# csyxwei/FFWM

Hardware: AMD Instinct MI355X
Metric: train img/s (128x128, full FFWM GAN step) (higher is better)
Workload: dtype f32; 1 GPU; BASELINE configs[2]: full FFWM train step (netG+netD+flowNetF+flowNetB, all losses, 3x Adam), synthetic MultiPIE-shaped 128x128; batch_per_gpu=8, global_batch=8, parallelism=dp1, grad_buckets=10, bucket_MiB=64

## Files before the change

### ffwm_amd/_lib.py

```python
import ctypes
import os

_HERE = os.path.dirname(os.path.abspath(__file__))
LIB_PATH = os.path.join(_HERE, "lib", "libffwm_hip.so")

F32, F64 = 0, 1
ABI_VERSION = 5

_lib = None

_p = ctypes.c_void_p
_i64 = ctypes.c_int64
_i = ctypes.c_int

_SIGNATURES = {
    "ffwm_block_extractor_forward": [_p, _p, _p] + [_i64] * 6 + [_i, _i, _p],
    "ffwm_block_extractor_backward": [_p, _p, _p, _p, _p] + [_i64] * 6 + [_i, _i, _p],
    "ffwm_block_extractor_backward_strided": [_p, _p, _p, ctypes.POINTER(_i64), _p, _p] + [_i64] * 6 + [_i, _i, _p],
    "ffwm_local_attn_reshape_backward_strided": [_p, ctypes.POINTER(_i64), _p] + [_i64] * 3 + [_i, _i, _i, _p],
    "ffwm_resample2d_backward_strided": [_p, _p, _p, ctypes.POINTER(_i64), _p, _p] + [_i64] * 6 + [_i, _i, _i, _i, _p],
    "ffwm_bn_lrelu_forward": [_p] * 9 + [_i64] * 3 + [ctypes.c_double] * 3 + [_i, _p],
    "ffwm_bn_lrelu_backward": [_p] * 10 + [_i64] * 3 + [ctypes.c_double] + [_i, _p],
    "ffwm_bn_res_act_forward": [_p] * 11 + [_i64] * 3 + [ctypes.c_double] * 3 + [_i, _i, _p],
    "ffwm_bn_res_act_backward": [_p] * 11 + [_i64] * 3 + [ctypes.c_double] + [_i, _i, _p],
    "ffwm_mfm_forward": [_p, _p, _p] + [_i64] * 3 + [_i, _p],
    "ffwm_mfm_backward": [_p, _p, _p, _p] + [_i64] * 3 + [_i, _p],
    "ffwm_add_act_forward": [_p, _p, _p, _i64, _i, ctypes.c_double, _i, _p],
    "ffwm_add_act_backward": [_p, _p, _p, _i64, _i, ctypes.c_double, _i, _p],
    "ffwm_sigmoid_gate_forward": [_p, _p, _p, _p, _p, _i64, _i, _p],
    "ffwm_sigmoid_gate_backward": [_p, _p, _p, _p, _p, _i64, _i, _p],
    "ffwm_bias_relu_forward": [_p, _p, _p] + [_i64] * 3 + [_i, _p],
    "ffwm_bias_act_forward": [_p, _p, _p, _p] + [_i64] * 5 + [_i, ctypes.c_double, _i, _p],
    "ffwm_flow_head_forward": [_p, _p, _p, _p] + [_i64] * 4 + [_i, _p],
    "ffwm_conv_thin_forward": [_p, _p, _p, _p] + [_i64] * 5 + [_i, ctypes.c_double, _i, _p],
    "ffwm_flow_up_forward": [_p, _p, _p, _p] + [_i64] * 4 + [_i, _p],
    "ffwm_flow_head_backward": [_p, _p, _p, _p, _p] + [_i64] * 4 + [_i, _p],
    "ffwm_flow_up_backward": [_p, _p, _p] + [_i64] * 4 + [_i, _p],
    "ffwm_conv2d_forward": [_p, _p, _p, _p, _p] + [_i64] * 5 + [_i, _i, _i, _i, _i64, _i64, _i, ctypes.c_double, _p, _i64, _i, _p],
    "ffwm_conv2d_wgrad": [_p, _p, _p] + [_i64] * 7 + [_i, _i, _i, _i, _p],
    "ffwm_conv2d_wgrad_tiled": [_p, _p, _p, _p] + [_i64] * 7 + [_i, _i, _i, _i, _i, _p],
    "ffwm_conv3x3_winograd_forward": [_p, _p, _p, _p, _p] + [_i64] * 5 + [_i, _i, ctypes.c_double, _i, _p],
    "ffwm_adam_step": [_p, _p, _p, _p, _i64] + [ctypes.c_double] * 4 + [_i64, _i, _p],
    "ffwm_adam_step_device": [_p, _p, _p, _p, _i64] + [ctypes.c_double] * 4 + [_p, _i, _p],
    "ffwm_conv3x3_wgrad": [_p, _p, _p, _p] + [_i64] * 5 + [_i, _p],
    "ffwm_conv3x3_wgrad_block": [_p, _p, _p, _p] + [_i64] * 9 + [_i, _p],
    "ffwm_block_attention_forward": [_p, _p, _p, _p] + [_i64] * 6 + [_i, _i, _p],
    "ffwm_block_attention_backward": [_p, _p, _p, _p, _p, _p, _p] + [_i64] * 6 + [_i, _i, _p],
    "ffwm_local_attn_reshape_forward": [_p, _p] + [_i64] * 3 + [_i, _i, _p],
    "ffwm_local_attn_reshape_backward": [_p, _p] + [_i64] * 3 + [_i, _i, _i, _p],
    "ffwm_resample2d_forward": [_p, _p, _p] + [_i64] * 6 + [_i, _i, _i, _p],
    "ffwm_resample2d_backward": [_p, _p, _p, _p, _p] + [_i64] * 6 + [_i, _i, _i, _i, _p],
    "ffwm_warp_forward": [_p, _p, _p] + [_i64] * 6 + [_i, _i, _p],
    "ffwm_warp_backward": [_p, _p, _p, _p, _p] + [_i64] * 6 + [_i, _i, _p],
    "ffwm_warp_multi_forward": [_p, _i, _i, _i, _p],
    "ffwm_warp_multi_backward": [_p, _i, _i, _i, _p],
    "ffwm_spectral_norm_forward": [_p, _i, _i, ctypes.c_double, _i, _p],
    "ffwm_spectral_norm_backward": [_p, _i, _i, _p],
    "ffwm_guided_filter_forward": [_p, _p, _p, _p, _i64, _i64, _i64, _i, ctypes.c_double, _i, _p],
    "ffwm_affine_regularization": [_p, _p, _p, _p, _i64, _i64, _i64, _i, ctypes.c_double, _i, _p],
    "ffwm_correlation_colmax": [_p, _p, _p, _i64, _i64, _i64, _i, _p],
    "ffwm_guided_filter_backward": [_p, _p, _p, _p, _p, _p, _i64, _i64, _i64, _i, _i, _p],
    "ffwm_l1_multi": [_p, _i, _p, _p, _i, _i, _p],
    "ffwm_conv3x3_winograd_weights_multi": [_p, _i, _i, _p],
    "ffwm_prof_enable": [_i],
    "ffwm_prof_collect": [],
    "ffwm_prof_get": [_i, ctypes.c_char_p, _i, ctypes.POINTER(_i64), ctypes.POINTER(ctypes.c_double),
                      ctypes.POINTER(ctypes.c_double)],
    "ffwm_prof_get_flops": [_i, ctypes.POINTER(ctypes.c_double)],
    "ffwm_prof_get_bound": [_i, ctypes.POINTER(ctypes.c_double)],
    "ffwm_prof_reset": [],
    "ffwm_set_option": [ctypes.c_char_p, _i],
    "ffwm_zero_fill": [_p, _i64, _p],
    "ffwm_abi_version": [],
}

EXPORTS = sorted(list(_SIGNATURES) + ["ffwm_last_error", "ffwm_conv3x3_winograd_workspace_bytes", "ffwm_conv3x3_winograd_splits",
                                      "ffwm_conv2d_forward_workspace"])


class FFWMError(RuntimeError):
    pass


def load():
    global _lib
    if _lib is not None:
        return _lib
    if not os.path.exists(LIB_PATH):
        raise FFWMError(
            "libffwm_hip.so is missing (%s). The HIP extension is the only implementation of the "
            "ffwm_amd ops -- build it with `python -m ffwm_amd.build`." % LIB_PATH)
    lib = ctypes.CDLL(LIB_PATH)
    for name, argtypes in _SIGNATURES.items():
        fn = getattr(lib, name)
        fn.argtypes = argtypes
        fn.restype = _i
    lib.ffwm_conv3x3_winograd_workspace_bytes.argtypes = [_i64, _i64]
    lib.ffwm_conv3x3_winograd_workspace_bytes.restype = _i64
    lib.ffwm_conv3x3_winograd_splits.argtypes = [_i64, _i64, _i64, _i64, _i64, _i]
    lib.ffwm_conv3x3_winograd_splits.restype = _i
    lib.ffwm_conv2d_forward_workspace.argtypes = [_i64] * 5 + [_i] * 4
    lib.ffwm_conv2d_forward_workspace.restype = _i64
    lib.ffwm_last_error.argtypes = []
    lib.ffwm_last_error.restype = ctypes.c_char_p
    got = lib.ffwm_abi_version()
    if got != ABI_VERSION:
        raise FFWMError("libffwm_hip.so ABI version %d, expected %d: rebuild it" % (got, ABI_VERSION))
    _lib = lib
    for kv in filter(None, os.environ.get("FFWM_OPTS", "").split(",")):
        k, _, v = kv.partition("=")
        if lib.ffwm_set_option(k.strip().encode(), int(v)) < 0:
            raise FFWMError("FFWM_OPTS: unknown option %r (or a negative value)" % k)
    return lib


def check(rc, what):
    if rc != 0:
        msg = load().ffwm_last_error()
        raise FFWMError("%s failed (status %d): %s" % (what, rc, msg.decode() if msg else "?"))


def prof_enable(on=True):
    return load().ffwm_prof_enable(1 if on else 0)


def prof_reset():
    load().ffwm_prof_reset()


def prof_collect():
    lib = load()
    n = lib.ffwm_prof_collect()
    rows = {}
    for i in range(n):
        name = ctypes.create_string_buffer(128)
        launches = _i64()
        ms = ctypes.c_double()
        nbytes = ctypes.c_double()
        check(lib.ffwm_prof_get(i, name, 128, ctypes.byref(launches), ctypes.byref(ms),
                                ctypes.byref(nbytes)), "ffwm_prof_get")
        flops = ctypes.c_double()
        check(lib.ffwm_prof_get_flops(i, ctypes.byref(flops)), "ffwm_prof_get_flops")
        bound = ctypes.c_double()
        check(lib.ffwm_prof_get_bound(i, ctypes.byref(bound)), "ffwm_prof_get_bound")
        k = max(launches.value, 1)
        rows[name.value.decode()] = {"launches": launches.value, "total_ms": ms.value,
                                     "avg_ms": ms.value / k, "bytes_per_launch": nbytes.value / k,
                                     "flops_per_launch": flops.value / k, "roofline_ms": bound.value}
    return rows


def set_option(key, value):
    rc = load().ffwm_set_option(key.encode(), int(value))
    if rc < 0:
        check(rc, "ffwm_set_option")
    return rc
```

### ffwm_amd/nets.py

```python
import math
import os

import torch
import torch.nn as nn
import torch.nn.functional as F
from torch.nn.utils import spectral_norm

from . import _ext
from . import conv as _conv
from .external_function import WarpFlipCat, WarpNet, warp_many

LRELU = 0.2


def _msra(mods):
    for m in mods:
        if isinstance(m, (nn.Conv2d, nn.ConvTranspose2d)):
            nn.init.kaiming_normal_(m.weight)
            if m.bias is not None:
                nn.init.constant_(m.bias, 0)


def _cbl(cin, cout, stride=1):
    return nn.Sequential(nn.Conv2d(cin, cout, 3, stride, 1, bias=True), nn.BatchNorm2d(cout),
                         nn.LeakyReLU(LRELU, inplace=True))


def _dbl(cin, cout):
    return nn.Sequential(nn.ConvTranspose2d(cin, cout, 4, 2, 1, bias=True), nn.BatchNorm2d(cout),
                         nn.LeakyReLU(LRELU, inplace=True))


def _flow_head(cin):
    return nn.Sequential(nn.Conv2d(cin, 2, 3, 1, 1, bias=True), nn.Tanh())


class FlowNet(nn.Module):

    def __init__(self, ngf=64, in_ch=3, keep_unused=True):
        super().__init__()
        g = ngf
        enc = [("conv0", in_ch, g, 1), ("conv1", g, g, 2), ("conv1_1", g, 2 * g, 1),
               ("conv2", 2 * g, 2 * g, 2), ("conv2_1", 2 * g, 2 * g, 1), ("conv3", 2 * g, 4 * g, 2),
               ("conv3_1", 4 * g, 4 * g, 1), ("conv4", 4 * g, 8 * g, 2), ("conv4_1", 8 * g, 8 * g, 1),
               ("conv5", 8 * g, 8 * g, 2), ("conv5_1", 8 * g, 8 * g, 1), ("conv6", 8 * g, 16 * g, 2),
               ("conv6_1", 16 * g, 16 * g, 1)]
        for name, cin, cout, s in enc:
            setattr(self, name, _cbl(cin, cout, s))
        cat = {5: 16 * g + 2, 4: 12 * g + 2, 3: 6 * g + 2, 2: g + 2, 1: g // 2 + 2, 0: g // 4 + 2}
        dec_out = {5: 8 * g, 4: 4 * g, 3: 2 * g, 2: g, 1: g // 2, 0: g // 4}
        dec_in = {5: 16 * g, 4: cat[5], 3: cat[4], 2: cat[3], 1: cat[2], 0: cat[1]}
        for L in range(5, -1, -1):
            setattr(self, "deconv%d" % L, _dbl(dec_in[L], dec_out[L]))
        for L in range(5, -1, -1):
            setattr(self, "inter_conv%d" % L, _cbl(cat[L], dec_out[L]))
        if keep_unused:
            for L in range(5, -1, -1):
                setattr(self, "inter_conv_occ%d" % L, _cbl(cat[L] - 1, dec_out[L]))
        heads = {6: 16 * g, 5: 8 * g, 4: 4 * g, 3: 2 * g, 2: g, 1: g // 2, 0: g // 4}
        for L in range(6, -1, -1):
            setattr(self, "predict_flow%d" % L, _flow_head(heads[L]))
        for L in range(6, 0, -1):
            setattr(self, "upsampled_flow%d_to_%d" % (L, L - 1), nn.ConvTranspose2d(2, 2, 4, 2, 1))
        _msra(self.modules())

    def unused_parameters(self):
        return [p for n, p in self.named_parameters() if n.startswith("inter_conv_occ")]

    def forward(self, x):
        f = self.conv0(x)
        skips = {}
        for L in range(1, 7):
            f = getattr(self, "conv%d_1" % L)(getattr(self, "conv%d" % L)(f))
            skips[L] = f
        flow = self.predict_flow6(f)
        flows = {}
        cat = None
        for L in range(5, -1, -1):
            up = getattr(self, "upsampled_flow%d_to_%d" % (L + 1, L))(flow)
            d = getattr(self, "deconv%d" % L)(f if L == 5 else cat)
            cat = torch.cat((skips[L], d, up) if L >= 3 else (d, up), 1)
            flow = getattr(self, "predict_flow%d" % L)(getattr(self, "inter_conv%d" % L)(cat))
            flows[L] = flow
        return flows[0], flows[1], flows[2]


class Tanh2(nn.Module):
    def forward(self, x):
        return (torch.tanh(x) + 1) / 2


def _activ(name):
    table = {"relu": nn.ReLU, "lrelu": lambda: nn.LeakyReLU(LRELU), "sigmoid": nn.Sigmoid, "tanh": nn.Tanh,
             "tanh2": Tanh2}
    if name not in table:
        raise NotImplementedError("Activation %s not implemented" % name)
    return table[name]()


def _sn(m, on):
    return spectral_norm(m) if on else m


class ResidualBlock(nn.Module):

    def __init__(self, inc, outc=None, kernel=3, activ="lrelu", sn=True):
        super().__init__()
        outc = inc if outc is None else outc
        pad = kernel // 2 if sn else kernel
        self.activ = _activ(activ)
        self.input = _sn(nn.Conv2d(inc, outc, 1, 1, 0), sn)
        self.blocks = nn.Sequential(_sn(nn.Conv2d(inc, outc, kernel, 1, pad), sn), nn.BatchNorm2d(outc),
                                    nn.LeakyReLU(LRELU), _sn(nn.Conv2d(outc, outc, kernel, 1, pad), sn),
                                    nn.BatchNorm2d(outc))

    def forward(self, x):
        return self.activ(self.blocks(x) + self.input(x))


class FusedResidualBlock(ResidualBlock):

    def forward(self, x):
        from .norm import RES_ACTS, bn_res_act, bn_res_act_ok
        from .residual import _act_of, add_act
        blocks, inp = self.blocks, self.input
        bn = blocks[-1] if isinstance(blocks, nn.Sequential) and len(blocks) >= 2 else None
        act, slope = _act_of(self.activ)
        if (bn is not None and isinstance(inp, nn.Conv2d) and not inp._forward_pre_hooks and not inp._forward_hooks
                and bn_res_act_ok(bn, x, RES_ACTS.get(act)) and torch.is_grad_enabled()):
            h = x
            for m in list(blocks)[:-1]:
                h = m(h)
            s = inp._conv_forward(x, inp.weight, None)
            if h.shape == s.shape and h.shape[1] == bn.num_features:
                return bn_res_act(h, bn, s, inp.bias, RES_ACTS[act], slope)
            return add_act(bn(h), s if inp.bias is None else s + inp.bias.view(1, -1, 1, 1), self.activ)
        return add_act(blocks(x), inp(x), self.activ)


def _conv_block(inc, outc, ks, s, p, activ="lrelu", res=0, bn=True, sn=True):
    layers = [_sn(nn.Conv2d(inc, outc, ks, s, p), sn)]
    if bn:
        layers.append(nn.BatchNorm2d(outc))
    if activ is not None:
        layers.append(_activ(activ))
    layers += [ResidualBlock(outc, activ=activ, sn=sn) for _ in range(res)]
    return nn.Sequential(*layers)


def _shuffle_block(inc, outc, sn=True):
    return nn.Sequential(_sn(nn.Conv2d(inc, outc * 4, 3, 1, 1), sn), nn.PixelShuffle(2), nn.BatchNorm2d(outc),
                         _activ("lrelu"))


class FFWM(nn.Module):

    def __init__(self, num_layers=3, isflip=True, sn=True, warp_flipcat=None):
        super().__init__()
        ch = [64, 64, 128, 256]
        dch = [256, 128, 64, 64]
        self.isflip = isflip
        dm = 3 if isflip else 2
        am = dm - 1
        self.layers = num_layers
        self.e0 = _conv_block(3, ch[0], 7, 1, 3, res=1, bn=False, sn=sn)
        for i in (1, 2, 3):
            setattr(self, "e%d" % i, _conv_block(ch[i - 1], ch[i], 4, 2, 1, res=1, sn=sn))
        d_in = [dch[0], dch[1] * dm, dch[2] * dm + 3]
        r_ch = [dch[1] * dm, dch[2] * dm + 3, dch[3] * dm + 3]
        for i in range(3):
            setattr(self, "d%d" % i, _shuffle_block(d_in[i], dch[i + 1], sn=sn))
        for i in range(3):
            setattr(self, "dres%d" % i, nn.Sequential(*[ResidualBlock(r_ch[i], activ="lrelu", sn=sn) for _ in range(2)]))
        for i in range(3):
            setattr(self, "rec%d" % i, _conv_block(r_ch[i], 3, 3, 1, 1, bn=False, activ="sigmoid", sn=sn))
        for i, c in enumerate((ch[2] * am, ch[1] * am, ch[0] * am)):
            setattr(self, "att%d" % i, nn.Sequential(_conv_block(c, c, 3, 1, 1, sn=sn),
                                                     ResidualBlock(c, c, activ="sigmoid", sn=sn)))
        self.warpNet = WarpNet()
        self._fused = warp_flipcat if warp_flipcat is not None else WarpFlipCat()
        self._multi = warp_flipcat is None and os.environ.get("FFWM_WARP_MULTI", "1") != "0"
        self.fuse_gate = False

    def _skip(self, feat, flow):
        if self.isflip:
            return self._fused(feat, flow)
        return self.warpNet(feat, flow)

    def _skips(self, enc, flow):
        feats = [enc[self.layers - 1 - i] for i in range(self.layers)]
        if self._multi and feats[0].is_cuda:
            return warp_many(feats, [flow[i] for i in range(self.layers)], self.isflip)
        return [self._skip(f, flow[i]) for i, f in enumerate(feats)]

    def forward(self, x, flow=None, return_att=False):
        enc = [self.e0(x)]
        for i in range(1, self.layers + 1):
            enc.append(getattr(self, "e%d" % i)(enc[-1]))
        fdec = enc[-1]
        recons, att = [], None
        if callable(flow):
            flow = flow()
        skips = self._skips(enc, flow) if self._multi else None
        for i in range(self.layers):
            dec = getattr(self, "d%d" % i)(fdec)
            skip = skips[i] if skips is not None else self._skip(enc[self.layers - 1 - i], flow[i])
            if self.fuse_gate:
                from .residual import gated
                skip, att = gated(getattr(self, "att%d" % i), skip)
            else:
                att = getattr(self, "att%d" % i)(skip)
                skip = skip * att
            parts = [skip, dec]
            if recons:
                parts.append(F.interpolate(recons[-1], scale_factor=2, mode="bilinear"))
            fdec = getattr(self, "dres%d" % i)(torch.cat(parts, 1))
            recons.append(getattr(self, "rec%d" % i)(fdec))
        out = (recons[-3], recons[-2], recons[-1])
        return out + (att,) if return_att else out


class WarpAttention(nn.Module):

    LEVELS = ((128, 32), (64, 64), (64, 128))

    def __init__(self, sn=True, warp_flipcat=None):
        super().__init__()
        for i, (c, _) in enumerate(self.LEVELS):
            setattr(self, "att%d" % i, nn.Sequential(_conv_block(2 * c, 2 * c, 3, 1, 1, sn=sn),
                                                     ResidualBlock(2 * c, 2 * c, activ="sigmoid", sn=sn)))
        self._fused = warp_flipcat if warp_flipcat is not None else WarpFlipCat()
        self._multi = warp_flipcat is None
        self.fuse_gate = False

    def forward(self, feats, flows):
        if self._multi and feats[0].is_cuda:
            skips = warp_many(list(feats), list(flows), True)
        else:
            skips = [self._fused(feat, flow) for feat, flow in zip(feats, flows)]
        if self.fuse_gate:
            from .residual import gated
            return [gated(getattr(self, "att%d" % i), skip)[0] for i, skip in enumerate(skips)]
        return [skip * getattr(self, "att%d" % i)(skip) for i, skip in enumerate(skips)]


class MSDiscriminator(nn.Module):

    def __init__(self, real_crop_size=128, inc=3, max_n_scales=9, scale_factor=2, base_channels=64, sigmoid=False):
        super().__init__()
        self.scale_factor = scale_factor
        n = int(math.ceil(math.log(real_crop_size / 16.0) / math.log(scale_factor)))
        self.max_n_scales = min(n, max_n_scales)
        self.nets = nn.ModuleList(self._make(inc, base_channels, sigmoid) for _ in range(self.max_n_scales))

    @staticmethod
    def _make(inc, c, sigmoid):
        layers = []
        for cin, cout in ((inc, c), (c, 2 * c), (2 * c, 4 * c)):
            layers += [spectral_norm(nn.Conv2d(cin, cout, 3, 2, 1)), nn.BatchNorm2d(cout), nn.LeakyReLU(LRELU, True)]
        if sigmoid:
            layers += [spectral_norm(nn.Conv2d(4 * c, 1, 1)), nn.Sigmoid()]
        else:
            layers += [nn.Conv2d(4 * c, 1, 1)]
        return nn.Sequential(*layers)

    def forward(self, x):
        total = self.nets[0](x)
        size = total.shape[2:]
        for i, net in enumerate(self.nets[1:5], start=1):
            small = F.interpolate(x, scale_factor=self.scale_factor ** (-i), mode="bilinear")
            total = total + F.interpolate(net(small), size=size, mode="bilinear")
        return total


FUSED_ACTIVATIONS = os.environ.get("FFWM_FUSED_ACT", "1") != "0"


_WINOGRAD_MFM = os.environ.get("FFWM_WINOGRAD_MFM", "0") == "1"


class mfm(nn.Module):

    def __init__(self, cin, cout, k=3, s=1, p=1, type=1):
        super().__init__()
        self.out_channels = cout
# ... 152 lines not shown
```

### ffwm_amd/norm.py

```python
import os

import torch
import torch.nn as nn
import torch.nn.functional as F
from torch.autograd import Function

from . import _ext, _lib


def _launch(fn_name, x, *args):
    dev = x.device.index
    cur = torch.cuda.current_device()
    if cur != dev:
        torch.cuda.set_device(dev)
    try:
        fn = getattr(_lib.load(), fn_name)
        _lib.check(fn(*args, _lib.F32, torch.cuda.current_stream(dev).cuda_stream), fn_name)
    finally:
        if cur != dev:
            torch.cuda.set_device(cur)


def _p(t):
    return None if t is None else t.data_ptr()


_SCRATCH = {}


def _scratch(x):
    C = x.shape[1]
    if C < 512 and x.numel() // C >= 32768:
        key = (x.device, C, torch.cuda.current_stream(x.device).cuda_stream)
        buf = _SCRATCH.get(key)
        if buf is None:
            buf = _SCRATCH[key] = torch.zeros(2 * C + (C + 1) // 2, device=x.device, dtype=torch.float64)
        return buf
    return None


def reset_scratch():
    _SCRATCH.clear()
    ext = _ext.get()
    if ext is not None and hasattr(ext, "bn_scratch_reset"):
        ext.bn_scratch_reset()


class _BnLreluFunction(Function):
    @staticmethod
    def forward(ctx, x, weight, bias, running_mean, running_var, eps, momentum, slope):
        B, C, H, W = x.shape
        y = torch.empty_like(x)
        save_mean = torch.empty(C, device=x.device, dtype=torch.float32)
        save_invstd = torch.empty(C, device=x.device, dtype=torch.float32)
        scratch = _scratch(x)
        _launch("ffwm_bn_lrelu_forward", x, _p(x), _p(weight), _p(bias), _p(running_mean), _p(running_var), _p(y),
                _p(save_mean), _p(save_invstd), _p(scratch), B, C, H * W, float(eps), float(momentum), float(slope))
        ctx.save_for_backward(x, weight, bias, save_mean, save_invstd)
        ctx.slope = float(slope)
        return y

    @staticmethod
    def backward(ctx, grad_y):
        x, weight, bias, save_mean, save_invstd = ctx.saved_tensors
        B, C, H, W = x.shape
        go = grad_y.contiguous()
        need_x, need_w, need_b = ctx.needs_input_grad[0], ctx.needs_input_grad[1], ctx.needs_input_grad[2]
        dx = torch.empty_like(x) if need_x else None
        dw = torch.empty(C, device=x.device, dtype=torch.float32) if (need_w and weight is not None) else None
        db = torch.empty(C, device=x.device, dtype=torch.float32) if (need_b and bias is not None) else None
        scratch = _scratch(x)
        _launch("ffwm_bn_lrelu_backward", x, _p(x), _p(go), _p(weight), _p(bias), _p(save_mean), _p(save_invstd), _p(dx),
                _p(dw), _p(db), _p(scratch), B, C, H * W, ctx.slope)
        return dx, dw, db, None, None, None, None, None


def _launch_act(fn_name, x, act, *args):
    dev = x.device.index
    cur = torch.cuda.current_device()
    if cur != dev:
        torch.cuda.set_device(dev)
    try:
        fn = getattr(_lib.load(), fn_name)
        _lib.check(fn(*args, int(act), _lib.F32, torch.cuda.current_stream(dev).cuda_stream), fn_name)
    finally:
        if cur != dev:
            torch.cuda.set_device(cur)


class _BnResActFunction(Function):

    @staticmethod
    def forward(ctx, x, weight, bias, running_mean, running_var, res, rbias, eps, momentum, slope, act):
        B, C, H, W = x.shape
        y = torch.empty_like(x)
        save_mean = torch.empty(C, device=x.device, dtype=torch.float32)
        save_invstd = torch.empty(C, device=x.device, dtype=torch.float32)
        scratch = _scratch(x)
        _launch_act("ffwm_bn_res_act_forward", x, act, _p(x), _p(weight), _p(bias), _p(running_mean), _p(running_var), _p(res), _p(rbias),
                    _p(y), _p(save_mean), _p(save_invstd), _p(scratch), B, C, H * W, float(eps), float(momentum), float(slope))
        ctx.save_for_backward(x, weight, save_mean, save_invstd, y)
        ctx.slope, ctx.act = float(slope), int(act)
        ctx.has_bias, ctx.has_rbias = bias is not None, rbias is not None
        return y

    @staticmethod
    @torch.autograd.function.once_differentiable
    def backward(ctx, grad_y):
        x, weight, save_mean, save_invstd, y = ctx.saved_tensors
        B, C, H, W = x.shape
        go = grad_y.contiguous()
        need = ctx.needs_input_grad
        dx = torch.empty_like(x) if need[0] else None
        dres = torch.empty_like(x) if need[5] else None
        dw = torch.empty(C, device=x.device, dtype=torch.float32) if (need[1] and weight is not None) else None
        want_db = (need[2] and ctx.has_bias) or (need[6] and ctx.has_rbias)
        db = torch.empty(C, device=x.device, dtype=torch.float32) if want_db else None
        scratch = _scratch(x)
        _launch_act("ffwm_bn_res_act_backward", x, ctx.act, _p(x), _p(y), _p(go), _p(weight), _p(save_mean), _p(save_invstd), _p(dx), _p(dres),
                    _p(dw), _p(db), _p(scratch), B, C, H * W, ctx.slope)
        return (dx, dw, db if (need[2] and ctx.has_bias) else None, None, None, dres, db if (need[6] and ctx.has_rbias) else None,
                None, None, None, None)


RES_ACTS = {"lrelu": 0, "sigmoid": 1}
_BN_RES = os.environ.get("FFWM_BN_RES_ACT", "1") != "0"


def bn_res_act_ok(bn, x, act_code):
    return (_BN_RES and act_code is not None and type(bn) in (nn.BatchNorm2d, HostCountBatchNorm2d) and bn.training and bn.momentum is not None and torch.is_tensor(x)
            and x.is_cuda and x.dtype == torch.float32 and x.dim() == 4 and x.numel() // x.shape[1] > 1 and not torch.is_autocast_enabled()
            and (bn.weight is None or bn.weight.dtype == torch.float32))


def bn_res_act(x, bn, res, rbias, act_code, slope):
    if bn.track_running_stats and bn.num_batches_tracked is not None:
        if hasattr(bn, "flush_batch_counter"):
            bn._pending_batches += 1
        else:
            bn.num_batches_tracked.add_(1)
    rm = bn.running_mean if bn.track_running_stats else None
    rv = bn.running_var if bn.track_running_stats else None
    return _BnResActFunction.apply(x.contiguous(), bn.weight, bn.bias, rm, rv, res.contiguous(), rbias, bn.eps, bn.momentum, slope, act_code)


MIN_FUSED_NUMEL = 1 << 20


MIN_FUSED_NUMEL_EXT = int(os.environ.get("FFWM_BN_MIN_NUMEL", str(1 << 20)))


def _kernel_ok(x):
    floor = MIN_FUSED_NUMEL if (MIN_FUSED_NUMEL == 0 or _ext.get() is None) else MIN_FUSED_NUMEL_EXT
    return (x.is_cuda and x.dtype == torch.float32 and x.dim() == 4 and x.numel() >= floor and x.is_contiguous()
            and x.data_ptr() % 16 == 0)


class BatchNormLeakyReLU2d(nn.BatchNorm2d):

    negative_slope = 0.2
    _pending_batches = 0

    def forward(self, x):
        if (self.training and self.momentum is not None and _kernel_ok(x)
                and (self.weight is None or self.weight.dtype == torch.float32)):
            if self.track_running_stats and self.num_batches_tracked is not None:
                self._pending_batches += 1
            rm = self.running_mean if self.track_running_stats else None
            rv = self.running_var if self.track_running_stats else None
            ext = _ext.get()
            if ext is not None:
                return ext.bn_lrelu(x, self.weight, self.bias, rm, rv, self.eps, self.momentum, self.negative_slope)
            return _BnLreluFunction.apply(x, self.weight, self.bias, rm, rv, self.eps, self.momentum, self.negative_slope)
        return F.leaky_relu(_bn_host_counted(self, x), self.negative_slope)

    def flush_batch_counter(self):
        if self._pending_batches and self.num_batches_tracked is not None:
            self.num_batches_tracked += self._pending_batches
        self._pending_batches = 0


def _bn_host_counted(m, x):
    if m.training and m.momentum is not None and m.track_running_stats and m.num_batches_tracked is not None and x.is_cuda:
        m._pending_batches += 1
        return F.batch_norm(x, m.running_mean, m.running_var, m.weight, m.bias, True, m.momentum, m.eps)
    return nn.BatchNorm2d.forward(m, x)


class HostCountBatchNorm2d(nn.BatchNorm2d):

    _pending_batches = 0

    def forward(self, x):
        return _bn_host_counted(self, x)

    def flush_batch_counter(self):
        if self._pending_batches and self.num_batches_tracked is not None:
            self.num_batches_tracked += self._pending_batches
        self._pending_batches = 0


def _flush_hook(module, *args, **kwargs):
    module.flush_batch_counter()


def _reset_hook(module, *args, **kwargs):
    module._pending_batches = 0


def fuse_bn_lrelu(net):
    n = 0
    for seq in [m for m in net.modules() if isinstance(m, nn.Sequential)]:
        keys = list(seq._modules.keys())
        for ka, kb in zip(keys, keys[1:]):
            a, b = seq._modules[ka], seq._modules[kb]
            if type(a) is nn.BatchNorm2d and type(b) is nn.LeakyReLU:
                a.__class__ = BatchNormLeakyReLU2d
                a.negative_slope = b.negative_slope
                a._pending_batches = 0
                a.register_state_dict_pre_hook(_flush_hook)
                a.register_load_state_dict_pre_hook(_reset_hook)
                seq._modules[kb] = nn.Identity()
                n += 1
    for m in net.modules():
        if type(m) is nn.BatchNorm2d:
            m.__class__ = HostCountBatchNorm2d
            m._pending_batches = 0
            m.register_state_dict_pre_hook(_flush_hook)
            m.register_load_state_dict_pre_hook(_reset_hook)
    return n
```

### include/ffwm_hip.h

```cpp
#ifndef FFWM_HIP_H_
#define FFWM_HIP_H_

#include <stdint.h>

#ifdef __cplusplus
extern "C" {
#endif

#define FFWM_ABI_VERSION 5

typedef enum {
    FFWM_OK = 0,
    FFWM_ERR_ARG = -1,
    FFWM_ERR_DTYPE = -2,
    FFWM_ERR_SIZE = -3,
    FFWM_ERR_LAUNCH = -4
} ffwm_status;

typedef enum { FFWM_F32 = 0, FFWM_F64 = 1 } ffwm_dtype;

int ffwm_abi_version(void);
const char* ffwm_last_error(void);

int ffwm_block_extractor_forward(const void* source, const void* flow_field, void* output,
                                 int64_t B, int64_t C, int64_t Hs, int64_t Ws, int64_t Hf,
                                 int64_t Wf, int kernel_size, int dtype, void* stream);

int ffwm_block_extractor_backward(const void* source, const void* flow_field,
                                  const void* grad_output, void* grad_source,
                                  void* grad_flow_field, int64_t B, int64_t C, int64_t Hs,
                                  int64_t Ws, int64_t Hf, int64_t Wf, int kernel_size,
                                  int dtype, void* stream);

int ffwm_local_attn_reshape_forward(const void* inputs, void* output, int64_t B, int64_t H,
                                    int64_t W, int kernel_size, int dtype, void* stream);

int ffwm_local_attn_reshape_backward(const void* grad_output, void* grad_inputs, int64_t B,
                                     int64_t H, int64_t W, int kernel_size, int accumulate,
                                     int dtype, void* stream);

int ffwm_block_extractor_backward_strided(const void* source, const void* flow_field, const void* grad_output,
                                          const int64_t* grad_output_strides, void* grad_source, void* grad_flow_field, int64_t B,
                                          int64_t C, int64_t Hs, int64_t Ws, int64_t Hf, int64_t Wf, int kernel_size, int dtype,
                                          void* stream);
int ffwm_local_attn_reshape_backward_strided(const void* grad_output, const int64_t* grad_output_strides, void* grad_inputs, int64_t B,
                                             int64_t H, int64_t W, int kernel_size, int accumulate, int dtype, void* stream);
int ffwm_resample2d_backward_strided(const void* input1, const void* input2, const void* grad_output,
                                     const int64_t* grad_output_strides, void* grad_input1, void* grad_input2, int64_t B, int64_t C,
                                     int64_t Hi, int64_t Wi, int64_t H, int64_t W, int kernel_size, int dilation,
                                     int reference_quirk, int dtype, void* stream);

int ffwm_resample2d_forward(const void* input1, const void* input2, void* output, int64_t B,
                            int64_t C, int64_t Hi, int64_t Wi, int64_t H, int64_t W,
                            int kernel_size, int dilation, int dtype, void* stream);

int ffwm_resample2d_backward(const void* input1, const void* input2, const void* grad_output,
                             void* grad_input1, void* grad_input2, int64_t B, int64_t C,
                             int64_t Hi, int64_t Wi, int64_t H, int64_t W, int kernel_size,
                             int dilation, int reference_quirk, int dtype, void* stream);

int ffwm_warp_forward(const void* feat, const void* flow, void* output, int64_t B, int64_t C,
                      int64_t Hi, int64_t Wi, int64_t H, int64_t W, int flipcat, int dtype,
                      void* stream);

int ffwm_warp_backward(const void* feat, const void* flow, const void* grad_output,
                       void* grad_feat, void* grad_flow, int64_t B, int64_t C, int64_t Hi,
                       int64_t Wi, int64_t H, int64_t W, int flipcat, int dtype, void* stream);

typedef struct ffwm_warp_problem {
    const void* feat;
    const void* flow;
    void* output;
    const void* grad_output;
    void* grad_feat;
    void* grad_flow;
    int64_t B, C, Hi, Wi, H, W;
} ffwm_warp_problem;
int ffwm_warp_multi_forward(const ffwm_warp_problem* problems, int n, int flipcat, int dtype, void* stream);
int ffwm_warp_multi_backward(const ffwm_warp_problem* problems, int n, int flipcat, int dtype, void* stream);

typedef struct ffwm_l1_problem {
    const void* x;
    const void* y;
    const void* mask;
    void* grad_x;
    int64_t n, chw, hw;
    double scale;
    int slot;
} ffwm_l1_problem;
int ffwm_l1_multi(const ffwm_l1_problem* problems, int n, void* out, const void* grad_out, int n_slots, int dtype, void* stream);

#define FFWM_SN_MAX_LAYERS 32
typedef struct {
    const void* weight;
    void* u;
    void* v;
    void* wv;
    void* weight_sn;
    void* sigma;
    void* u_saved;
    void* v_saved;
    int rows, cols;
} ffwm_sn_layer;

int ffwm_spectral_norm_forward(const ffwm_sn_layer* layers, int n_layers, int power_iterations,
                               double eps, int dtype, void* stream);

typedef struct {
    const void* weight;
    const void* u;
    const void* v;
    const void* sigma;
    const void* grad_weight_sn;
    void* grad_weight;
    void* partials;
    int rows, cols;
} ffwm_sn_grad_layer;

int ffwm_spectral_norm_backward(const ffwm_sn_grad_layer* layers, int n_layers, int dtype,
                                void* stream);

int ffwm_guided_filter_forward(const void* x, const void* y, void* output, void* saved,
                               int64_t planes, int64_t H, int64_t W, int r, double eps, int dtype,
                               void* stream);

int ffwm_guided_filter_backward(const void* x, const void* y, const void* saved,
                                const void* grad_output, void* grad_x, void* workspace,
                                int64_t planes, int64_t H, int64_t W, int r, int dtype, void* stream);

int ffwm_affine_regularization(const void* flow, const void* ktk, void* loss_sum, void* grad_flow,
                               int64_t B, int64_t h, int64_t w, int kernel_size, double loss_scale,
                               int dtype, void* stream);

int ffwm_correlation_colmax(const void* source, const void* target, void* out, int64_t B, int64_t N,
                            int64_t C, int dtype, void* stream);

int ffwm_block_attention_forward(const void* source, const void* flow_field, const void* weights, void* output,
                                 int64_t B, int64_t C, int64_t Hs, int64_t Ws, int64_t Hf, int64_t Wf,
                                 int kernel_size, int dtype, void* stream);

int ffwm_block_attention_backward(const void* source, const void* flow_field, const void* weights,
                                  const void* grad_output, void* grad_source, void* grad_flow_field,
                                  void* grad_weights, int64_t B, int64_t C, int64_t Hs, int64_t Ws, int64_t Hf,
                                  int64_t Wf, int kernel_size, int dtype, void* stream);

int ffwm_conv3x3_wgrad(const void* input, const void* grad_output, void* grad_weight, void* grad_bias, int64_t B,
                       int64_t C, int64_t K, int64_t H, int64_t W, int dtype, void* stream);

int ffwm_conv3x3_wgrad_block(const void* input, const void* grad_output, void* grad_weight, void* grad_bias, int64_t B,
                             int64_t C, int64_t K, int64_t H, int64_t W, int64_t k_begin, int64_t k_end, int64_t c_begin,
                             int64_t c_end, int dtype, void* stream);

int ffwm_bn_lrelu_forward(const void* x, const void* weight, const void* bias, void* running_mean, void* running_var,
                          void* y, void* save_mean, void* save_invstd, void* scratch, int64_t B, int64_t C, int64_t HW,
                          double eps, double momentum, double negative_slope, int dtype, void* stream);

int ffwm_bn_lrelu_backward(const void* x, const void* grad_out, const void* weight, const void* bias,
                           const void* save_mean, const void* save_invstd, void* grad_x, void* grad_weight,
                           void* grad_bias, void* scratch, int64_t B, int64_t C, int64_t HW, double negative_slope,
                           int dtype, void* stream);

int ffwm_bn_res_act_forward(const void* x, const void* weight, const void* bias, void* running_mean, void* running_var,
                            const void* res, const void* rbias, void* y, void* save_mean, void* save_invstd, void* scratch,
                            int64_t B, int64_t C, int64_t HW, double eps, double momentum, double negative_slope, int act,
                            int dtype, void* stream);
int ffwm_bn_res_act_backward(const void* x, const void* y, const void* grad_out, const void* weight, const void* save_mean,
                             const void* save_invstd, void* grad_x, void* grad_res, void* grad_weight, void* grad_bias,
                             void* scratch, int64_t B, int64_t C, int64_t HW, double negative_slope, int act, int dtype,
                             void* stream);

int ffwm_mfm_forward(const void* x, const void* bias, void* y, int64_t B, int64_t C, int64_t HW, int dtype, void* stream);
int ffwm_mfm_backward(const void* x, const void* bias, const void* grad_y, void* grad_x, int64_t B, int64_t C, int64_t HW,
                      int dtype, void* stream);

int ffwm_add_act_forward(const void* a, const void* b, void* y, int64_t n, int act, double negative_slope, int dtype, void* stream);
int ffwm_add_act_backward(const void* y, const void* grad_y, void* grad_z, int64_t n, int act, double negative_slope, int dtype,
                          void* stream);
int ffwm_sigmoid_gate_forward(const void* a, const void* b, const void* x, void* att, void* y, int64_t n, int dtype, void* stream);
int ffwm_sigmoid_gate_backward(const void* x, const void* att, const void* grad_y, void* grad_z, void* grad_x, int64_t n, int dtype,
                               void* stream);

int ffwm_bias_relu_forward(const void* h, const void* bias, void* y, int64_t B, int64_t C, int64_t HW, int dtype, void* stream);

int ffwm_bias_act_forward(const void* h, const void* bias, void* y, void* y2, int64_t B, int64_t C, int64_t HW,
                          int64_t y_batch_stride, int64_t y2_batch_stride, int act, double negative_slope, int dtype,
                          void* stream);
int ffwm_conv_thin_forward(const void* x, const void* weight_ctk, const void* bias, void* y, int64_t B, int64_t C, int64_t H, int64_t W,
                           int64_t K, int act, double negative_slope, int dtype, void* stream);

int ffwm_flow_head_forward(const void* x, const void* weight, const void* bias, void* y, int64_t B, int64_t C, int64_t H,
                           int64_t W, int dtype, void* stream);
int ffwm_flow_up_forward(const void* flow, const void* weight, const void* bias, void* out, int64_t B, int64_t H, int64_t W,
                         int64_t out_batch_stride, int dtype, void* stream);

int ffwm_flow_head_backward(const void* y, const void* grad_y, const void* weight, void* grad_z, void* grad_x, int64_t B, int64_t C,
                            int64_t H, int64_t W, int dtype, void* stream);
int ffwm_flow_up_backward(const void* grad_out, const void* weight, void* grad_x, int64_t B, int64_t H, int64_t W,
                          int64_t grad_out_batch_stride, int dtype, void* stream);

int64_t ffwm_conv2d_forward_workspace(int64_t B, int64_t C, int64_t H, int64_t W, int64_t K, int kernel, int stride, int pad,
                                      int transposed);
int ffwm_conv2d_forward(const void* input, const void* weight, const void* bias, void* output, void* output2, int64_t B, int64_t C,
                        int64_t H, int64_t W, int64_t K, int kernel, int stride, int pad, int transposed, int64_t out_batch_stride,
                        int64_t out2_batch_stride, int act, double negative_slope, void* workspace, int64_t workspace_bytes,
                        int dtype, void* stream);

int ffwm_conv2d_wgrad(const void* rows, const void* gathered, void* grad_weight, int64_t B, int64_t K, int64_t Ho, int64_t Wo,
                      int64_t C, int64_t H, int64_t W, int kernel, int stride, int pad, int dtype, void* stream);

int ffwm_conv2d_wgrad_tiled(const void* rows, const void* gathered, void* grad_weight, void* grad_bias, int64_t B, int64_t K,
                            int64_t Ho, int64_t Wo, int64_t C, int64_t H, int64_t W, int kernel, int stride, int pad, int prezeroed,
                            int dtype, void* stream);

int64_t ffwm_conv3x3_winograd_workspace_bytes(int64_t K, int64_t C);
int ffwm_conv3x3_winograd_splits(int64_t B, int64_t C, int64_t H, int64_t W, int64_t K, int act);

typedef struct ffwm_wino_weights {
    const void* weight;
    void* workspace;
    int64_t K, C;
    int data_gradient;
    int width_multiple_of_4;
} ffwm_wino_weights;
int ffwm_conv3x3_winograd_weights_multi(const ffwm_wino_weights* items, int n, int dtype, void* stream);
int ffwm_conv3x3_winograd_forward(const void* input, const void* weight, const void* bias, void* output, void* workspace,
                                  int64_t B, int64_t C, int64_t H, int64_t W, int64_t K, int data_gradient, int act,
                                  double slope, int dtype, void* stream);

int ffwm_adam_step(void* params, const void* grads, void* exp_avg, void* exp_avg_sq, int64_t n, double lr,
                   double beta1, double beta2, double eps, int64_t step, int dtype, void* stream);

int ffwm_adam_step_device(void* params, const void* grads, void* exp_avg, void* exp_avg_sq, int64_t n, double lr, double beta1,
                          double beta2, double eps, void* state, int dtype, void* stream);

int ffwm_prof_enable(int on);
int ffwm_prof_collect(void);
int ffwm_prof_get(int row, char* name, int name_len, int64_t* launches, double* total_ms,
                  double* algorithmic_bytes);
int ffwm_prof_get_flops(int row, double* algorithmic_flops);
int ffwm_prof_get_bound(int row, double* roofline_ms);
int ffwm_prof_reset(void);

int ffwm_set_option(const char* key, int value);

int ffwm_zero_fill(void* p, int64_t bytes, void* stream);

#ifdef __cplusplus
}
#endif
#endif
```

Before: 218.7 img/s.

## Fuse 1x1 shortcut conv into BN residual activation tail kernel

Adds a HIP kernel that computes the residual block's 1x1 shortcut convolution with MFMA instructions and applies batch-norm scale/shift, residual add and activation in the same pass. A separate stats kernel first reduces per-channel sums. The aim is to avoid materialising the shortcut conv output and the extra launch and memory traffic of a separate conv followed by bn_res_act. It is gated to blocks with 64 channels and enough pixel tiles. Backward reuses the existing bn_res_act backward plus a conv weight grad.

```diff
diff --git a/ffwm_amd/_lib.py b/ffwm_amd/_lib.py
--- a/ffwm_amd/_lib.py
+++ b/ffwm_amd/_lib.py
@@ -23,6 +23,7 @@
     "ffwm_bn_lrelu_backward": [_p] * 10 + [_i64] * 3 + [ctypes.c_double] + [_i, _p],
     "ffwm_bn_res_act_forward": [_p] * 11 + [_i64] * 3 + [ctypes.c_double] * 3 + [_i, _i, _p],
     "ffwm_bn_res_act_backward": [_p] * 11 + [_i64] * 3 + [ctypes.c_double] + [_i, _i, _p],
+    "ffwm_res_tail_forward": [_p] * 12 + [_i64] * 4 + [ctypes.c_double] * 3 + [_i, _i, _p],
     "ffwm_mfm_forward": [_p, _p, _p] + [_i64] * 3 + [_i, _p],
     "ffwm_mfm_backward": [_p, _p, _p, _p] + [_i64] * 3 + [_i, _p],
     "ffwm_add_act_forward": [_p, _p, _p, _i64, _i, ctypes.c_double, _i, _p],
@@ -75,7 +76,7 @@
 }
 
 EXPORTS = sorted(list(_SIGNATURES) + ["ffwm_last_error", "ffwm_conv3x3_winograd_workspace_bytes", "ffwm_conv3x3_winograd_splits",
-                                      "ffwm_conv2d_forward_workspace"])
+                                      "ffwm_conv2d_forward_workspace", "ffwm_res_tail_workspace"])
 
 
 class FFWMError(RuntimeError):
@@ -101,6 +102,8 @@
     lib.ffwm_conv3x3_winograd_splits.restype = _i
     lib.ffwm_conv2d_forward_workspace.argtypes = [_i64] * 5 + [_i] * 4
     lib.ffwm_conv2d_forward_workspace.restype = _i64
+    lib.ffwm_res_tail_workspace.argtypes = [_i64] * 3
+    lib.ffwm_res_tail_workspace.restype = _i64
     lib.ffwm_last_error.argtypes = []
     lib.ffwm_last_error.restype = ctypes.c_char_p
     got = lib.ffwm_abi_version()
diff --git a/ffwm_amd/csrc/residual_tail.hip b/ffwm_amd/csrc/residual_tail.hip
--- /dev/null
+++ b/ffwm_amd/csrc/residual_tail.hip
@@ -0,0 +1,227 @@
+#include "common.hpp"
+
+namespace ffwm {
+namespace {
+
+typedef float f32x16 __attribute__((ext_vector_type(16)));
+
+constexpr int kRtThreads = 256;
+constexpr int kRtPix = 128;
+constexpr int kRtCC = 16;
+constexpr int kRtMaxMT = 8;
+constexpr int kRtMaxK = 1024;
+constexpr int kRtStatThreads = 1024;
+
+struct RtGeo {
+    int B, C, K, HW, S;
+    float eps, momentum, slope;
+    int act;
+};
+
+__device__ __forceinline__ float rt_act(float v, float slope, int act) {
+    return act == 1 ? 1.f / (1.f + __expf(-v)) : (v > 0.f ? v : v * slope);
+}
+
+__global__ void __launch_bounds__(kRtStatThreads)
+rt_stats_kernel(const float* __restrict__ h, double* __restrict__ part, RtGeo g) {
+    __shared__ double red[2 * (kRtStatThreads / kWave)];
+    const int k = blockIdx.x, t = threadIdx.x;
+    const size_t cstride = static_cast<size_t>(g.K) * g.HW;
+    const float* hk = h + static_cast<size_t>(k) * g.HW;
+    double s = 0, ss = 0;
+    if (g.HW % 4 == 0) {
+        const int hw4 = g.HW / 4, all4 = g.B * hw4;
+        const int chunk = (all4 + g.S - 1) / g.S;
+        const int first = blockIdx.y * chunk, last = min(all4, first + chunk);
+        for (int j = first + t; j < last; j += kRtStatThreads) {
+            const int b = j / hw4, i = j - b * hw4;
+            const float4 v = *(reinterpret_cast<const float4*>(hk + b * cstride) + i);
+            s += (static_cast<double>(v.x) + static_cast<double>(v.y)) + (static_cast<double>(v.z) + static_cast<double>(v.w));
+            ss += (static_cast<double>(v.x) * v.x + static_cast<double>(v.y) * v.y) +
+                  (static_cast<double>(v.z) * v.z + static_cast<double>(v.w) * v.w);
+        }
+    } else {
+        const int all = g.B * g.HW;
+        const int chunk = (all + g.S - 1) / g.S;
+        const int first = blockIdx.y * chunk, last = min(all, first + chunk);
+        for (int j = first + t; j < last; j += kRtStatThreads) {
+            const int b = j / g.HW, i = j - b * g.HW;
+            const double v = hk[b * cstride + i];
+            s += v;
+            ss += v * v;
+        }
+    }
+    s = wave_sum(s);
+    ss = wave_sum(ss);
+    constexpr int NW = kRtStatThreads / kWave;
+    if ((t & (kWave - 1)) == 0) {
+        red[t / kWave] = s;
+        red[NW + t / kWave] = ss;
+    }
+    __syncthreads();
+    if (t == 0) {
+        double sa = 0, sb = 0;
+        for (int w = 0; w < NW; ++w) {
+            sa += red[w];
+            sb += red[NW + w];
+        }
+        part[(static_cast<size_t>(k) * g.S + blockIdx.y) * 2] = sa;
+        part[(static_cast<size_t>(k) * g.S + blockIdx.y) * 2 + 1] = sb;
+    }
+}
+
+template <int MT>
+__global__ void __launch_bounds__(kRtThreads)
+rt_fwd_kernel(const float* __restrict__ h, const float* __restrict__ x, const float* __restrict__ wsc, const float* __restrict__ gamma,
+              const float* __restrict__ beta, float* __restrict__ run_mean, float* __restrict__ run_var,
+              const float* __restrict__ rbias, const double* __restrict__ part, float* __restrict__ y,
+              float* __restrict__ save_mean, float* __restrict__ save_invstd, RtGeo g) {
+    constexpr int WROW = MT * 32 + 4;
+    __shared__ float sc[kRtMaxK], sh[kRtMaxK];
+    __shared__ float wl[kRtCC * WROW];
+    __shared__ float xl[kRtCC * kRtPix];
+    const int t = threadIdx.x, lane = t & (kWave - 1), wave = t / kWave;
+    const int b = blockIdx.y, p0 = blockIdx.x * kRtPix;
+
+    const double n = static_cast<double>(g.B) * g.HW;
+    for (int k = t; k < g.K; k += kRtThreads) {
+        double s = 0, ss = 0;
+        for (int i = 0; i < g.S; ++i) {
+            s += part[(static_cast<size_t>(k) * g.S + i) * 2];
+            ss += part[(static_cast<size_t>(k) * g.S + i) * 2 + 1];
+        }
+        const double mean = s / n;
+        double var = ss / n - mean * mean;
+        var = var > 0 ? var : 0;
+        const float invstd = static_cast<float>(1.0 / sqrt(var + static_cast<double>(g.eps)));
+        const float meanf = static_cast<float>(mean);
+        if (blockIdx.x == 0 && blockIdx.y == 0) {
+            save_mean[k] = meanf;
+            save_invstd[k] = invstd;
+            if (run_mean) {
+                const double unbiased = n > 1 ? var * n / (n - 1) : var;
+                run_mean[k] = (1.f - g.momentum) * run_mean[k] + g.momentum * meanf;
+                run_var[k] = (1.f - g.momentum) * run_var[k] + g.momentum * static_cast<float>(unbiased);
+            }
+        }
+        const float ga = gamma ? gamma[k] : 1.f, be = beta ? beta[k] : 0.f;
+        float shift = be - meanf * ga * invstd;
+        if (rbias) shift += rbias[k];
+        sc[k] = ga * invstd;
+        sh[k] = shift;
+    }
+
+    const float* xb = x + static_cast<size_t>(b) * g.C * g.HW;
+    const size_t ob = static_cast<size_t>(b) * g.K * g.HW;
+    const int nstage = (g.C + kRtCC - 1) / kRtCC;
+    const int px = wave * 32 + (lane & 31);
+    const int half = lane >> 5;
+
+    for (int k0 = 0; k0 < g.K; k0 += MT * 32) {
+        f32x16 acc[MT];
+#pragma unroll
+        for (int m = 0; m < MT; ++m)
+#pragma unroll
+            for (int r = 0; r < 16; ++r) acc[m][r] = 0.f;
+        float wr[2 * MT], xr[8];
+        auto fetch = [&](int c0) {
+#pragma unroll
+            for (int i = 0; i < 2 * MT; ++i) {
+                const int idx = t + kRtThreads * i;
+                const int k = k0 + idx / kRtCC, c = c0 + idx % kRtCC;
+                wr[i] = (k < g.K && c < g.C) ? wsc[static_cast<size_t>(k) * g.C + c] : 0.f;
+            }
+#pragma unroll
+            for (int i = 0; i < 8; ++i) {
+                const int idx = t + kRtThreads * i;
+                const int c = c0 + idx / kRtPix, p = p0 + idx % kRtPix;
+                xr[i] = (c < g.C && p < g.HW) ? xb[static_cast<size_t>(c) * g.HW + p] : 0.f;
+            }
+        };
+        fetch(0);
+        for (int st = 0; st < nstage; ++st) {
+            __syncthreads();
+#pragma unroll
+            for (int i = 0; i < 2 * MT; ++i) {
+                const int idx = t + kRtThreads * i;
+                wl[(idx % kRtCC) * WROW + idx / kRtCC] = wr[i];
+            }
+#pragma unroll
+            for (int i = 0; i < 8; ++i) xl[t + kRtThreads * i] = xr[i];
+            __syncthreads();
+            if (st + 1 < nstage) fetch((st + 1) * kRtCC);
+#pragma unroll
+            for (int q = 0; q < kRtCC / 2; ++q) {
+                const int c = 2 * q + half;
+                const float bv = xl[c * kRtPix + px];
+#pragma unroll
+                for (int m = 0; m < MT; ++m)
+                    acc[m] = __builtin_amdgcn_mfma_f32_32x32x2f32(wl[c * WROW + m * 32 + (lane & 31)], bv, acc[m], 0, 0, 0);
+            }
+        }
+        const int p = p0 + px;
+        if (p < g.HW) {
+#pragma unroll
+            for (int m = 0; m < MT; ++m) {
+                float hv[16];
+#pragma unroll
+                for (int r = 0; r < 16; ++r) {
+                    const int k = k0 + m * 32 + (r & 3) + 8 * (r >> 2) + 4 * half;
+                    hv[r] = k < g.K ? h[ob + static_cast<size_t>(k) * g.HW + p] : 0.f;
+                }
+#pragma unroll
+                for (int r = 0; r < 16; ++r) {
+                    const int k = k0 + m * 32 + (r & 3) + 8 * (r >> 2) + 4 * half;
+                    if (k < g.K) y[ob + static_cast<size_t>(k) * g.HW + p] = rt_act(hv[r] * sc[k] + sh[k] + acc[m][r], g.slope, g.act);
+                }
+            }
+        }
+    }
+}
+
+}
+}
+
+using namespace ffwm;
+
+static int rt_slices(int64_t B, int64_t K, int64_t HW) {
+    int64_t S = (1024 + K - 1) / K;
+    const int64_t cap = B * HW / 4096;
+    if (S > cap) S = cap;
+    if (S > 32) S = 32;
+    return S < 1 ? 1 : static_cast<int>(S);
+}
+
+extern "C" int64_t ffwm_res_tail_workspace(int64_t B, int64_t K, int64_t HW) {
+    if (B <= 0 || K <= 0 || HW <= 0) return 0;
+    return 2 * K * rt_slices(B, K, HW) * static_cast<int64_t>(sizeof(double));
+}
+
+extern "C" int ffwm_res_tail_forward(const void* h, const void* x, const void* shortcut_weight, const void* weight, const void* bias,
+                                     void* running_mean, void* running_var, const void* rbias, void* y, void* save_mean,
+                                     void* save_invstd, void* workspace, int64_t B, int64_t C, int64_t K, int64_t HW, double eps,
+                                     double momentum, double negative_slope, int act, int dtype, void* stream) {
+    const char* fn = "ffwm_res_tail_forward";
+    FFWM_REQUIRE(dtype == FFWM_F32, FFWM_ERR_DTYPE, "%s: float32 only", fn);
+    FFWM_REQUIRE(B > 0 && C > 0 && K > 0 && HW > 0 && B * HW > 1, FFWM_ERR_ARG, "%s: need B, C, K, H*W > 0 and more than one value per channel", fn);
+    FFWM_REQUIRE(K <= kRtMaxK && B < 65536 && B * K * HW < (1LL << 31) && B * C * HW < (1LL << 31), FFWM_ERR_SIZE, "%s: tensor too large", fn);
+    FFWM_REQUIRE(h && x && shortcut_weight && y && save_mean && save_invstd && workspace, FFWM_ERR_ARG, "%s: NULL tensor pointer", fn);
+    FFWM_REQUIRE(act == 0 || act == 1, FFWM_ERR_ARG, "%s: act must be 0 (leaky relu) or 1 (sigmoid)", fn);
+    FFWM_REQUIRE((running_mean == nullptr) == (running_var == nullptr), FFWM_ERR_ARG, "%s: running_mean and running_var go together", fn);
+    RtGeo g{(int)B, (int)C, (int)K, (int)HW, rt_slices(B, K, HW), (float)eps, (float)momentum, (float)negative_slope, act};
+    hipStream_t st = static_cast<hipStream_t>(stream);
+    LaunchScope ls("res_tail_fwd", st, 4.0 * (3.0 * B * K * HW + 1.0 * B * C * HW + 1.0 * K * C), 2.0 * B * HW * C * K);
+    hipLaunchKernelGGL(rt_stats_kernel, dim3((unsigned)K, (unsigned)g.S), dim3(kRtStatThreads), 0, st, (const float*)h, (double*)workspace, g);
+    const int tiles = static_cast<int>((K + 31) / 32);
+    const int passes = (tiles + kRtMaxMT - 1) / kRtMaxMT;
+    const int mt = (tiles + passes - 1) / passes;
+    const dim3 grid((unsigned)((HW + kRtPix - 1) / kRtPix), (unsigned)B);
+    const bool ok = dispatch<1, 2, 3, 4, 5, 6, 7, 8>(mt, [&](auto MT) {
+        hipLaunchKernelGGL((rt_fwd_kernel<decltype(MT)::value>), grid, dim3(kRtThreads), 0, st, (const float*)h, (const float*)x,
+                           (const float*)shortcut_weight, (const float*)weight, (const float*)bias, (float*)running_mean,
+                           (float*)running_var, (const float*)rbias, (const double*)workspace, (float*)y, (float*)save_mean,
+                           (float*)save_invstd, g);
+    });
+    if (!ok) return no_kernel(fn);
+    return check_launch(fn);
+}
diff --git a/ffwm_amd/nets.py b/ffwm_amd/nets.py
--- a/ffwm_amd/nets.py
+++ b/ffwm_amd/nets.py
@@ -121,7 +121,7 @@
 class FusedResidualBlock(ResidualBlock):
 
     def forward(self, x):
-        from .norm import RES_ACTS, bn_res_act, bn_res_act_ok
+        from .norm import RES_ACTS, bn_res_act, bn_res_act_ok, res_tail, res_tail_ok
         from .residual import _act_of, add_act
         blocks, inp = self.blocks, self.input
         bn = blocks[-1] if isinstance(blocks, nn.Sequential) and len(blocks) >= 2 else None
@@ -131,6 +131,10 @@
             h = x
             for m in list(blocks)[:-1]:
                 h = m(h)
+            if (inp.kernel_size == (1, 1) and inp.stride == (1, 1) and inp.padding == (0, 0) and inp.dilation == (1, 1) and inp.groups == 1
+                    and h.dim() == 4 and h.shape[1] == bn.num_features == inp.out_channels and res_tail_ok(h, x, inp.weight)):
+                from .conv import OwnBwdConv2d
+                return res_tail(h, bn, x, inp.weight, inp.bias, RES_ACTS[act], slope, isinstance(inp, OwnBwdConv2d))
             s = inp._conv_forward(x, inp.weight, None)
             if h.shape == s.shape and h.shape[1] == bn.num_features:
                 return bn_res_act(h, bn, s, inp.bias, RES_ACTS[act], slope)
diff --git a/ffwm_amd/norm.py b/ffwm_amd/norm.py
--- a/ffwm_amd/norm.py
+++ b/ffwm_amd/norm.py
@@ -142,6 +142,85 @@
     rm = bn.running_mean if bn.track_running_stats else None
     rv = bn.running_var if bn.track_running_stats else None
     return _BnResActFunction.apply(x.contiguous(), bn.weight, bn.bias, rm, rv, res.contiguous(), rbias, bn.eps, bn.momentum, slope, act_code)
+
+
+class _ResTailFunction(Function):
+
+    @staticmethod
+    def forward(ctx, h, x, sweight, weight, bias, running_mean, running_var, rbias, eps, momentum, slope, act, own_wgrad):
+        B, K, H, W = h.shape
+        C = x.shape[1]
+        y = torch.empty_like(h)
+        save_mean = torch.empty(K, device=h.device, dtype=torch.float32)
+        save_invstd = torch.empty(K, device=h.device, dtype=torch.float32)
+        lib = _lib.load()
+        part = torch.empty(lib.ffwm_res_tail_workspace(B, K, H * W) // 8, device=h.device, dtype=torch.float64)
+        _launch_act("ffwm_res_tail_forward", h, act, _p(h), _p(x), _p(sweight), _p(weight), _p(bias), _p(running_mean), _p(running_var),
+                    _p(rbias), _p(y), _p(save_mean), _p(save_invstd), _p(part), B, C, K, H * W, float(eps), float(momentum), float(slope))
+        ctx.save_for_backward(h, x, sweight, weight, save_mean, save_invstd, y)
+        ctx.slope, ctx.act, ctx.own_wgrad = float(slope), int(act), bool(own_wgrad)
+        ctx.has_bias, ctx.has_rbias = bias is not None, rbias is not None
+        return y
+
+    @staticmethod
+    @torch.autograd.function.once_differentiable
+    def backward(ctx, grad_y):
+        from .conv import conv_weight_grad
+        h, x, sweight, weight, save_mean, save_invstd, y = ctx.saved_tensors
+        B, K, H, W = h.shape
+        go = grad_y.contiguous()
+        need = ctx.needs_input_grad
+        dh = torch.empty_like(h) if need[0] else None
+        dres = torch.empty_like(h) if (need[1] or need[2]) else None
+        dw = torch.empty(K, device=h.device, dtype=torch.float32) if (need[3] and weight is not None) else None
+        want_db = (need[4] and ctx.has_bias) or (need[7] and ctx.has_rbias)
+        db = torch.empty(K, device=h.device, dtype=torch.float32) if want_db else None
+        _launch_act("ffwm_bn_res_act_backward", h, ctx.act, _p(h), _p(y), _p(go), _p(weight), _p(save_mean), _p(save_invstd), _p(dh), _p(dres),
+                    _p(dw), _p(db), _scratch_ptr(h), B, K, H * W, ctx.slope)
+        gx = gw = None
+        w4 = sweight.view(K, x.shape[1], 1, 1)
+        if need[2] and ctx.own_wgrad:
+            gw = conv_weight_grad(x, dres, w4, 1, 0, False)[0].view_as(sweight)
+        if need[1] or (need[2] and gw is None):
+            gx, gw2, _ = torch.ops.aten.convolution_backward(dres, x, w4, None, [1, 1], [0, 0], [1, 1], False, [0, 0], 1,
+                                                             [bool(need[1]), bool(need[2] and gw is None), False])
+            if gw is None and need[2]:
+                gw = gw2.view_as(sweight)
+        return (dh, gx, gw, dw, db if (need[4] and ctx.has_bias) else None, None, None, db if (need[7] and ctx.has_rbias) else None,
+                None, None, None, None, None)
+
+
+def _scratch_ptr(x):
+    return _p(_scratch(x))
+
+
+RES_TAIL_MIN_TILES = 512
+RES_TAIL_MIN_CHANNELS = 64
+RES_TAIL_MAX_CHANNELS = 64
+_RES_TAIL = os.environ.get("FFWM_RES_TAIL", "1") != "0"
+
+
+def res_tail_ok(h, x, sweight):
+    if not (_RES_TAIL and torch.is_tensor(x) and x.is_cuda and x.dtype == torch.float32 and x.dim() == 4 and x.is_contiguous()
+            and h.is_contiguous() and sweight.dtype == torch.float32 and sweight.is_contiguous() and sweight.dim() == 4
+            and sweight.shape[2:] == (1, 1) and x.shape[0] == h.shape[0] and x.shape[2:] == h.shape[2:]
+            and x.shape[1] == sweight.shape[1] and h.shape[1] == sweight.shape[0]):
+        return False
+    B, K, H, W = h.shape
+    C = x.shape[1]
+    return (min(C, K) >= RES_TAIL_MIN_CHANNELS and max(C, K) <= RES_TAIL_MAX_CHANNELS and B * ((H * W + 127) // 128) >= RES_TAIL_MIN_TILES
+            and max(h.numel(), x.numel()) < (1 << 31))
+
+
+def res_tail(h, bn, x, sweight, rbias, act_code, slope, own_wgrad):
+    if bn.track_running_stats and bn.num_batches_tracked is not None:
+        if hasattr(bn, "flush_batch_counter"):
+            bn._pending_batches += 1
+        else:
+            bn.num_batches_tracked.add_(1)
+    rm = bn.running_mean if bn.track_running_stats else None
+    rv = bn.running_var if bn.track_running_stats else None
+    return _ResTailFunction.apply(h, x, sweight, bn.weight, bn.bias, rm, rv, rbias, bn.eps, bn.momentum, slope, act_code, own_wgrad)
 
 
 MIN_FUSED_NUMEL = 1 << 20
diff --git a/include/ffwm_hip.h b/include/ffwm_hip.h
--- a/include/ffwm_hip.h
+++ b/include/ffwm_hip.h
@@ -169,6 +169,12 @@
                              void* scratch, int64_t B, int64_t C, int64_t HW, double negative_slope, int act, int dtype,
                              void* stream);
 
+int64_t ffwm_res_tail_workspace(int64_t B, int64_t K, int64_t HW);
+int ffwm_res_tail_forward(const void* h, const void* x, const void* shortcut_weight, const void* weight, const void* bias,
+                          void* running_mean, void* running_var, const void* rbias, void* y, void* save_mean, void* save_invstd,
+                          void* workspace, int64_t B, int64_t C, int64_t K, int64_t HW, double eps, double momentum,
+                          double negative_slope, int act, int dtype, void* stream);
+
 int ffwm_mfm_forward(const void* x, const void* bias, void* y, int64_t B, int64_t C, int64_t HW, int dtype, void* stream);
 int ffwm_mfm_backward(const void* x, const void* bias, const void* grad_y, void* grad_x, int64_t B, int64_t C, int64_t HW,
                       int dtype, void* stream);
```

Result: slower. 214.0 img/s (-2.1%).
